# toutane/arcanefem

Measured on AMD Instinct MI355X. Metric: MDoF/s assembly + CG iter/s, Poisson-3D P1 at 1/2/4/8 MI355X, higher is better.
Workload: dtype f64; 1 GPU; C2 Poisson-3D P1; n=215, dof_total=10077696, nnz_rank0=150048286, parallelism=z-slab x1, RCCL halo + all-reduce in CG

## Files before the change

arcanefem_amd/_capi.py:

```python
from __future__ import annotations

import ctypes
import os

_HERE = os.path.dirname(os.path.abspath(__file__))
LIB_PATH = os.environ.get("AFEM_LIB") or os.path.join(_HERE, "libafem.so")

AFEM_OK = 0
AFEM_MEM_HOST = 0
AFEM_MEM_DEVICE = 1
AFEM_RHS_ADD = 0
AFEM_RHS_SET = 1
AFEM_SOLVER_AUTO = 0
AFEM_SOLVER_PCG = 1
AFEM_SOLVER_DIRECT = 2
AFEM_NEUMANN_VALUE = 0
AFEM_NEUMANN_NORMAL = 1
AFEM_NEUMANN_TRACTION = 2
UNIQUE_ID_BYTES = 128
ERRORS = {1: "ArgumentException", 2: "HipError", 3: "NotImplementedException", 4: "StateError",
          5: "NotFound", 6: "CommError", 7: "LimitExceeded"}


class AfemError(RuntimeError):
# ... 25 lines not shown
                ("coords", ctypes.c_void_p), ("rows", ctypes.c_void_p), ("columns", ctypes.c_void_p),
                ("values", ctypes.c_void_p), ("error_flag", ctypes.c_void_p), ("stream", ctypes.c_void_p)]


class FunctorPlan(ctypes.Structure):
    _fields_ = [("n_units", ctypes.c_int64), ("n_stages", ctypes.c_int64), ("n_entries", ctypes.c_int64),
                ("rows_per_layer", ctypes.c_int32), ("width", ctypes.c_int32), ("nbuf", ctypes.c_int32),
                ("wide", ctypes.c_int32), ("block_size", ctypes.c_int32), ("nb_node_per_cell", ctypes.c_int32),
                ("ordered_per_block", ctypes.c_int32), ("lattice", ctypes.c_int32), ("units", ctypes.c_void_p),
                ("stage_ptr", ctypes.c_void_p), ("layer_rows", ctypes.c_void_p), ("entries", ctypes.c_void_p),
                ("entries2", ctypes.c_void_p), ("rows", ctypes.c_void_p), ("values", ctypes.c_void_p),
                ("stream", ctypes.c_void_p), ("patterns", ctypes.c_void_p), ("n_patterns", ctypes.c_int64),
                ("packed", ctypes.c_int32), ("reserved0", ctypes.c_int32)]


class Csr32View(ctypes.Structure):
    _fields_ = [("n_rows", ctypes.c_int64), ("nnz", ctypes.c_int64), ("rows", ctypes.c_void_p),
                ("rows_nb_column", ctypes.c_void_p), ("columns", ctypes.c_void_p), ("values", ctypes.c_void_p),
                ("identity", ctypes.c_int32)]


class BsrStats(ctypes.Structure):
    _fields_ = [("n_incidences", ctypes.c_int64), ("inc_table_entries", ctypes.c_int64),
                ("max_row_len", ctypes.c_int32), ("rows_per_block", ctypes.c_int32), ("max_seg", ctypes.c_int64),
                ("max_slice_nodes", ctypes.c_int32), ("max_slice_width", ctypes.c_int32),
                ("n_slices", ctypes.c_int64), ("brick_order", ctypes.c_int32), ("uniform_slices", ctypes.c_int32),
                ("last_kernel", ctypes.c_int32), ("stencil_slices", ctypes.c_int32),
                ("stencil_sig", ctypes.c_int32), ("shared_strip_slices", ctypes.c_int64),
                ("uniform_instance_slices", ctypes.c_int64), ("general_slices", ctypes.c_int64),
                ("cube_lattice", ctypes.c_int32), ("cube_axes", ctypes.c_int32),
                ("cube_row_stride", ctypes.c_int64), ("cube_units", ctypes.c_int64),
                ("cube_unit_records", ctypes.c_int64), ("cube_unit_table", ctypes.c_void_p),
                ("cube_xcd_cost_spread", ctypes.c_double), ("cube_sched", ctypes.c_int32),
                ("reserved0", ctypes.c_int32)]


class SolverOpts(ctypes.Structure):
    _fields_ = [("method", ctypes.c_int32), ("max_iter", ctypes.c_int32), ("rtol", ctypes.c_double),
                ("atol", ctypes.c_double), ("check_every", ctypes.c_int32), ("fixed_iterations", ctypes.c_int32),
                ("initial_guess", ctypes.c_int32), ("precond_block", ctypes.c_int32), ("multigrid", ctypes.c_int32),
                ("profile_comm", ctypes.c_int32), ("amg", ctypes.c_int32)]


class SolveStats(ctypes.Structure):
    _fields_ = [("iterations", ctypes.c_int32), ("converged", ctypes.c_int32), ("rel_residual", ctypes.c_double),
                ("residual_norm", ctypes.c_double), ("solve_ms", ctypes.c_double), ("spmv_kernel", ctypes.c_int32),
                ("halo_wait_ms", ctypes.c_double), ("allreduce_ms", ctypes.c_double), ("halo_bytes", ctypes.c_int64),
                ("n_halo", ctypes.c_int32), ("n_allreduce", ctypes.c_int32), ("amg_levels", ctypes.c_int32),
                ("amg_coarse_rows", ctypes.c_int64), ("amg_complexity", ctypes.c_double),
                ("amg_setup_ms", ctypes.c_double), ("precond_ms", ctypes.c_double)]


class StepTiming(ctypes.Structure):
    _fields_ = [("assemble_ms", ctypes.c_double), ("rhs_ms", ctypes.c_double), ("bc_ms", ctypes.c_double),
                ("solve_ms", ctypes.c_double), ("precond_ms", ctypes.c_double), ("update_ms", ctypes.c_double),
                ("total_ms", ctypes.c_double), ("iterations", ctypes.c_int32), ("reserved0", ctypes.c_int32),
                ("nnz_blocks", ctypes.c_int64), ("n_incidences", ctypes.c_int64), ("n_nodes", ctypes.c_int64),
                ("n_own_nodes", ctypes.c_int64)]


ALLREDUCE_FN = ctypes.CFUNCTYPE(ctypes.c_int, ctypes.c_void_p, ctypes.POINTER(ctypes.c_double), ctypes.c_int64)
EXCHANGE_FN = ctypes.CFUNCTYPE(ctypes.c_int, ctypes.c_void_p, ctypes.c_int, ctypes.POINTER(ctypes.c_int32),
                               ctypes.POINTER(ctypes.c_double), ctypes.POINTER(ctypes.c_int64),
                               ctypes.POINTER(ctypes.c_double), ctypes.POINTER(ctypes.c_int64))


class HostTransport(ctypes.Structure):
# ... 144 lines not shown
```

arcanefem_amd/csrc/afem_internal.hpp:

```cpp
#pragma once

#include <hip/hip_runtime.h>

#include <cstdint>
#include <map>
#include <memory>
#include <stdexcept>
#include <string>
#include <thread>
#include <utility>
#include <vector>

#include "../../include/arcanefem_amd.h"

namespace afem {

#ifndef AFEM_NT_STORES
#define AFEM_NT_STORES 0
#endif
template <class T>
__device__ __forceinline__ void st_out(T* p, T v)
{
#if AFEM_NT_STORES
  __builtin_nontemporal_store(v, p);
// ... 165 lines not shown
  int64_t n_msl = 0;
  int msl_nodes = 0;
  int ms_nodes = 0, mb_nodes = 0, mb_w = 0;
  int u_nodes = 0, u_w = 0;
  DevBuf<SliceRec> rec_k, rec_ur;
  DevBuf<uint8_t> urslot;
  DevBuf<SliceRec> rec_k0, rec_u1;
  DevBuf<uint8_t> u1slot;
  int64_t n_k0 = 0, n_u1 = 0;
  int64_t n_k = 0, n_ur = 0;
  int sig_k = -1, k_nodes = 0, ur_nodes = 0, ur_w = 0;
  int64_t n_strip_shared = 0;
  bool rec_ok = false;
  DevBuf<int64_t> pos_rb;
  DevBuf<uint32_t> pos_dl;
  DevBuf<unsigned long long> tickets;
  int64_t ticket_gen = 0;
  int64_t n_slices = 0;
  int64_t n_incidences = 0;
  int max_row_len = 0;
  int64_t max_wave_seg = 0;
  DevBuf<int64_t> diag_pos;
  bool canon = false;
  DevBuf<uint8_t> cperm;
  bool cube_ok = false;
  int64_t cube_L[3] = { 0, 0, 0 };
  bool cube_natural = false;
  int nat_axes[3] = { 0, 1, 2 };
  int64_t nat_L[3] = { 0, 0, 0 };
  int64_t cube_row_stride = 0;
  DevBuf<uint32_t> cube_units;
  int64_t cube_units_n = 0, cube_units_real = 0;
  int cube_units_sched = 0;
  double cube_xcd_spread = 0.0;
  int64_t cube_units_key[12] = { 0, 0, 0, 0, 0, 0, 0, 0, 0, 0, 0, 0 };
  DevBuf<int32_t> cube_phys;
  DevBuf<int64_t> cube_rb;
  DevBuf<uint64_t> cube_slot;
  DevBuf<int32_t> cube_lat;
  DevBuf<uint64_t> cube_pinv;
};

struct LinearSystem;

struct FunctorPlan {
  bool valid = false;
  int nb_dof = 0;
  int rl = 64, w = 0, nbuf = 1, wide = 0, lattice = 0;
  int fx = 0, fy = 0, zs = 1;
  int64_t n_units = 0, n_stages = 0, n_entries = 0, n_coalesced = 0;
  DevBuf<afem_functor_unit> units;
  DevBuf<int64_t> stage_ptr;
  DevBuf<int32_t> layer_rows;
  DevBuf<uint32_t> ent, ent2;
  int packed = 0;
  int64_t n_patterns = 0;
  DevBuf<uint32_t> patterns;
};
void functor_plan_build(struct Bsr& b);

struct HandOver {
  bool valid = false, identity = false;
  int64_t n_rows = 0, nnz = 0;
  DevBuf<int32_t> rows, rnc, cols;
  DevBuf<int64_t> src;
  DevBuf<double> vals;
};

// ... 232 lines not shown
```

arcanefem_amd/csrc/capi.cpp:

```cpp
#include <hip/hip_runtime.h>

#include <algorithm>
#include <cstring>
#include <string>
#include <vector>

#include <rocprofiler-sdk-roctx/roctx.h>

#include "afem_internal.hpp"

using namespace afem;

namespace {
thread_local std::string g_last_error;

int fail(int code, const char* msg)
{
  g_last_error = msg ? msg : "unknown error";
  return code;
}
}

#define API_BEGIN try {
#define API_END                                              \
// ... 634 lines not shown
  API_END
}

int afem_bsr_get_stats(afem_bsr* b, afem_bsr_stats* st)
{
  API_BEGIN
  NOT_NULL(b);
  NOT_NULL(st);
  AFEM_REQUIRE(b->has_sparsity, AFEM_ERR_STATE, "no sparsity");
  st->n_incidences = b->s.n_incidences;
  st->inc_table_entries = (int64_t)b->s.inc.n;
  st->max_row_len = b->s.max_row_len;
  st->rows_per_block = afem::assembly_uses_lds(*b) ? 64 : 0;
  st->max_seg = b->s.max_wave_seg;
  st->max_slice_nodes = b->s.max_slice_nodes;
  st->max_slice_width = b->s.max_slice_w;
  st->n_slices = b->s.n_slices;
  st->brick_order = b->s.lattice ? 2 : b->s.brick_order ? 1 : 0;
  st->cube_lattice = b->s.cube_natural ? 2 : (b->s.canon && b->s.cube_ok) ? 3
                     : (b->mesh->st.valid && b->mesh->st.dim == 3 && !b->s.canon) ? 1 : 0;
  st->uniform_slices = (int32_t)b->s.n_uni;
  st->stencil_slices = (int32_t)b->s.n_k;
  st->stencil_sig = b->s.sig_k;
  st->shared_strip_slices = b->s.n_strip_shared;
  st->uniform_instance_slices = b->s.n_ur;
  st->general_slices = b->s.n_ms + b->s.n_mb;
  st->cube_axes = b->s.cube_natural ? b->s.nat_axes[0] + 3 * b->s.nat_axes[1] + 9 * b->s.nat_axes[2] : 0;
  st->cube_row_stride = b->s.cube_row_stride;
  st->cube_units = b->s.cube_units_real;
  st->cube_unit_records = b->s.cube_units_n;
  st->cube_unit_table = b->s.cube_units.p;
  st->cube_xcd_cost_spread = b->s.cube_xcd_spread;
  st->cube_sched = b->s.cube_units_sched;
  st->reserved0 = 0;
  st->last_kernel = b->last_kernel;
  API_END
}

int afem_bsr_get_sizes(afem_bsr* b, int64_t* n_rows, int64_t* nnz)
{
  API_BEGIN
  NOT_NULL(b);
  AFEM_REQUIRE(b->has_sparsity, AFEM_ERR_STATE, "no sparsity");
  if (n_rows) *n_rows = b->s.n_rows * b->nb_dof;
  if (nnz) *nnz = b->s.nnz * b->nb_dof * b->nb_dof;
  API_END
}

int afem_bsr_download(afem_bsr* b, int64_t* rows, int32_t* cols, double* vals)
{
  API_BEGIN
  NOT_NULL(b);
  AFEM_REQUIRE(b->has_sparsity, AFEM_ERR_STATE, "no sparsity");
  Ctx& ctx = *b->mesh->ctx;
  ctx.set_device();
  if (rows) AFEM_HIP(hipMemcpyAsync(rows, b->s.row_ptr.p, b->s.row_ptr.bytes(), hipMemcpyDeviceToHost, ctx.stream));
  if (cols && b->s.nnz)
    AFEM_HIP(hipMemcpyAsync(cols, b->s.cols.p, (size_t)b->s.nnz * sizeof(int32_t), hipMemcpyDeviceToHost, ctx.stream));
  if (vals && b->values.n)
    AFEM_HIP(hipMemcpyAsync(vals, b->values.p, b->values.bytes(), hipMemcpyDeviceToHost, ctx.stream));
  ctx.sync();
  API_END
}

int afem_bsr_export_csr32(afem_bsr* b, int32_t* rows, int32_t* rows_nb_column, int32_t* columns, double* values)
{
  API_BEGIN
// ... 869 lines not shown
```

arcanefem_amd/csrc/cubes.hip:

```cpp
#include "afem_internal.hpp"

#include <algorithm>
#include <cstring>
#include <limits>
#include <vector>

#pragma clang diagnostic ignored "-Wpass-failed"

namespace afem {

namespace {

inline unsigned grid_for(int64_t n, int threads) { return (unsigned)((n + threads - 1) / threads); }

struct P3 {
  double x, y, z;
};
__device__ __forceinline__ P3 psub(P3 a, P3 b) { return P3{ a.x - b.x, a.y - b.y, a.z - b.z }; }
__device__ __forceinline__ P3 pcross(P3 a, P3 b)
{
  return P3{ fma(a.y, b.z, -(a.z * b.y)), fma(a.z, b.x, -(a.x * b.z)), fma(a.x, b.y, -(a.y * b.x)) };
}
__device__ __forceinline__ double pdot(P3 a, P3 b) { return fma(a.z, b.z, fma(a.y, b.y, a.x * b.x)); }
__device__ __forceinline__ double precip(double a)
// ... 99 lines not shown
constexpr int kCol = 9;
constexpr int kAcc = 15;

#ifndef AFEM_CUBES_WAVESYNC
#define AFEM_CUBES_WAVESYNC 1
#endif
__device__ __forceinline__ void wave_lds_order()
{
#if AFEM_CUBES_WAVESYNC
  __builtin_amdgcn_fence(__ATOMIC_ACQ_REL, "wavefront");
  __builtin_amdgcn_wave_barrier();
#else
  __syncthreads();
#endif
}

template <bool NT>
__device__ __forceinline__ void put(double* p, double v)
{
  if constexpr (NT)
    __builtin_nontemporal_store(v, p);
  else
    *p = v;
}

struct CubeCanon {
  const int32_t* phys;
  const int64_t* rb;
  const uint64_t* slot;
  double* stage;
};

constexpr int kCubesBase = 16 | 32 | 64 | 256 | 512 | 1024 | 2048;
constexpr int kCubesV = kCubesBase | 4096;

template <int STRIDE>
constexpr int cube_waves() { return STRIDE == 64 ? 2 : 3; }
template <int STRIDE, bool CARRY, bool XEX, bool YEX, bool CANON, bool HAS_RHS, bool RHS_ADD, int DIAG = kCubesV>
__global__ __launch_bounds__(64) __attribute__((amdgpu_waves_per_eu(cube_waves<STRIDE>(), cube_waves<STRIDE>()))) void k_assemble_cubes(
    CubeGeom g, const int64_t* __restrict__ rows, const double* __restrict__ coords, double* __restrict__ vals,
    double* __restrict__ rhs, CubeCanon cc)
{
  __shared__ __align__(16) double acc[2][kAcc][STRIDE];
  constexpr int NCZ = CARRY ? 1 : 2;
  __shared__ double cz[NCZ][3][kCol * kCol];
  const int lane = threadIdx.x;
  const uint2 rec = g.units[blockIdx.x];
  const int z0 = (int)(rec.y & 0xffffffu), z1 = z0 + (int)(rec.y >> 24);
  if (z0 >= z1) return;
  AFEM_CWT(0, __builtin_amdgcn_s_memrealtime());
  const int cx0 = kRun * (int)(rec.x & 0xffffu), cy0 = kRun * (int)(rec.x >> 16);
  const int zc_first = max(z0 - 1, 0);
  const int zc_last = min(z1 - 1, g.nzc - 1);

  const int ci = lane & 7, cj = lane >> 3;
  const int gx = cx0 - 1 + ci, gy = cy0 - 1 + cj;
  const bool cube_in = gx >= 0 && gy >= 0 && gx + 1 < g.npx && gy + 1 < g.npy;
  auto node_xy = [&](int q, int& nx, int& ny) {
    nx = cx0 - 1 + q % kCol;
    ny = cy0 - 1 + q / kCol;
  };
  double pre[2][3];
  int32_t pid[2] = { 0, 0 };
  auto layer_base = [&](int k) { return (int64_t)__builtin_amdgcn_readfirstlane(local_layer(g, k)) * g.L; };
  int64_t xy_id[2];
#pragma unroll
  for (int h = 0; h < 2; ++h) {
    const int q = min(lane + 64 * h, kCol * kCol - 1);
    int nx, ny;
    node_xy(q, nx, ny);
    nx = min(max(nx, 0), g.npx - 1);
    ny = min(max(ny, 0), g.npy - 1);
    xy_id[h] = nx + (int64_t)g.npx * ny;
  }
  auto clamp_layer = [&](int k) { return is_local(g, k) ? k : g.k0; };
  auto prefetch_ids = [&](int k) {
    if constexpr (CANON) {
      const int32_t* const lp = cc.phys + layer_base(clamp_layer(k));
#pragma unroll
      for (int h = 0; h < 2; ++h) pid[h] = lp[xy_id[h]];
    }
  };
  auto load_layer_to = [&](int k, double (&dst)[2][3]) {
    const double* const lc = CANON ? coords : coords + 3 * layer_base(clamp_layer(k));
#pragma unroll
    for (int h = 0; h < 2; ++h) {
      const int64_t n = CANON ? (int64_t)pid[h] : xy_id[h];
      dst[h][0] = lc[3 * n];
      dst[h][1] = lc[3 * n + 1];
      dst[h][2] = lc[3 * n + 2];
    }
  };
  auto load_layer = [&](int k) { load_layer_to(k, pre); };
  auto store_layer = [&](int buf) {
    buf = NCZ == 1 ? 0 : buf;
#pragma unroll
    for (int h = 0; h < 2; ++h) {
      const int q = min(lane + 64 * h, kCol * kCol - 1);
      cz[buf][0][q] = pre[h][0];
      cz[buf][1][q] = pre[h][1];
      cz[buf][2][q] = pre[h][2];
    }
  };
  constexpr bool DROWS = (DIAG & 256) != 0 && STRIDE == 64;
  constexpr bool SW = DROWS && CARRY && XEX && YEX && (DIAG & 2048) != 0 && (DIAG & 2) == 0;
  auto slot = [&](int b, int r, int o) -> double* {
    return SW ? &acc[b][0][0] + kAcc * r + o : &acc[b][o][r];
  };
  if (!SW || g.acc_init != g.acc_init) {
    const double fill = SW ? g.acc_init : 0.0;
    for (int i = lane; i < 2 * kAcc * STRIDE; i += 64) (&acc[0][0][0])[i] = fill;
  }

  const int rx = lane % kRun, ry = lane / kRun;
  const int nx = cx0 + rx, ny = cy0 + ry;
  const bool full_flush_on = g.full_flush != 0;
  constexpr bool STAGE = CANON && (DIAG & 1024) != 0;
  int64_t pf_rb = 0, pf_re = 0, pf_r = 0;
  uint64_t pf_slot = 0;
  double pf_rhs = 0.0;
  const int64_t row_xy = min(nx, g.npx - 1) + (int64_t)g.npx * min(ny, g.npy - 1);
  auto prefetch_rows = [&](int z) {
    const int zz = (z >= z0 && z < z1) ? z : z0;
    const int64_t lb = layer_base(zz);
    const int64_t li = lb + row_xy;
    if constexpr (STAGE) {
      (void)li;
    }
    else if constexpr (CANON) {
      pf_r = cc.phys[li];
      pf_rb = cc.rb[li];
      pf_slot = cc.slot[li];
    }
    else {
      pf_r = li;
      pf_rb = (rows + lb)[row_xy];
      pf_re = (rows + lb)[row_xy + 1];
      if constexpr (RHS_ADD) pf_rhs = rhs[pf_r];
    }
  };
  const bool xy_full = cx0 >= 1 && cx0 + kRun <= g.npx - 1 && cy0 >= 1 && cy0 + kRun <= g.npy - 1;
  auto full_range = [&](int zlo, int zhi, int& zf0, int& zf1) {
    const bool on = !CANON && xy_full && full_flush_on;
    zf0 = on ? min(max(zlo, g.k0 + 1), zhi) : zhi;
    zf1 = on ? max(min(zhi, g.nzc), zf0) : zhi;
  };
  constexpr bool RS = !CANON && (DIAG & 4096) != 0;
  int64_t rs_rb = 0;
  auto load_run_bases = [&](int z) {
    const int zz = (z >= z0 && z < z1) ? z : z0;
    rs_rb = (rows + layer_base(zz))[row_xy];
  };
  auto flush_full = [&](int z, double* const* sb) {
    const int b = z & 1;
    const int lr = min(lane, STRIDE - 1);
    double v[15];
    double sum = 0.0;
#pragma unroll
    for (int o = 0; o < 15; ++o) {
      v[o] = *slot(b, lr, o);
      if (o != 7) sum += v[o];
    }
    const double meas = v[7];
    v[7] = -sum;
    if constexpr (HAS_RHS) {
      const bool valid = lane < kRows;
      const double rv = RHS_ADD ? pf_rhs + g.f_meas * meas : g.f_meas * meas;
      const int64_t r0 = lane_i64(pf_r, 0);
      const double rv0 = lane_f64(rv, 0);
      put<(DIAG & 128) != 0>(&rhs[valid ? pf_r : r0], valid ? rv : rv0);
    }
    const int64_t rb = pf_rb;
    double* img = &acc[b][0][0];
    if constexpr (SW) {
      img[kAcc * lane + 7] = v[7];
    }
    else {
      wave_lds_order();
#pragma unroll
      for (int o = 0; o < 15; ++o) img[15 * (STRIDE == 64 ? lane : lr) + o] = v[o];
// ... 17 lines not shown
      }
      else if constexpr ((DIAG & 64) != 0) {
        const double a0 = ra[q][0], a1 = ra[q][1];
        typedef double d2u __attribute__((ext_vector_type(2), aligned(8)));
        if constexpr ((DIAG & 32) != 0)
          __builtin_nontemporal_store(d2u{ a0, a1 }, reinterpret_cast<d2u*>(&dst[t2]));
        else
          *reinterpret_cast<d2u*>(&dst[t2]) = d2u{ a0, a1 };
      }
      else if constexpr ((DIAG & 32) != 0) {
        __builtin_nontemporal_store(img[15 * kRun * q + lane], &dst[lane]);
        __builtin_nontemporal_store(img[15 * kRun * q + t1], &dst[t1]);
      }
      else {
        dst[lane] = img[15 * kRun * q + lane];
        dst[t1] = img[15 * kRun * q + t1];
      }
    }
    wave_lds_order();
    if constexpr (SW) {
    }
    else if constexpr ((kAcc * STRIDE) % 2 == 0) {
      double2* const img2 = reinterpret_cast<double2*>(img);
#pragma unroll
      for (int i = 0; i < (kAcc * STRIDE / 2 + 63) / 64; ++i)
        img2[min(64 * i + lane, kAcc * STRIDE / 2 - 1)] = make_double2(0.0, 0.0);
      wave_lds_order();
    }
    else {
#pragma unroll
      for (int i = 0; i < (kAcc * STRIDE + 63) / 64; ++i) img[min(64 * i + lane, kAcc * STRIDE - 1)] = 0.0;
      wave_lds_order();
    }
  };
  auto flush_stage = [&](int z) {
    const int b = z & 1;
    const bool valid = lane < kRows && nx < g.npx && ny < g.npy;
    uint32_t mask = 0;
#pragma unroll
    for (int o = 0; o < 15; ++o) {
      const int xx = nx + kOffX[o], yy = ny + kOffY[o], zz = z + kOffZ[o];
      const uint32_t in = (uint32_t)(xx >= 0) & (uint32_t)(yy >= 0) & (uint32_t)(xx < g.npx) & (uint32_t)(yy < g.npy) &
                          (uint32_t)(zz >= 0) & (uint32_t)(zz <= g.nzc);
      mask |= in << o;
    }
    if (!valid) mask = 0;
    double v[15];
    double sum = 0.0;
    const int lr = min(lane, STRIDE - 1);
#pragma unroll
    for (int o = 0; o < 15; ++o) {
      v[o] = *slot(b, lr, o);
      if (o != 7 && ((mask >> o) & 1u)) sum += v[o];
    }
    const double meas = v[7];
    v[7] = -sum;
    wave_lds_order();
    double* img = &acc[b][0][0];
    if (lane < kRows) {
#pragma unroll
      for (int o = 0; o < 15; ++o) img[16 * lane + o] = (!SW || o == 7 || ((mask >> o) & 1u)) ? v[o] : 0.0;
      img[16 * lane + 15] = meas;
    }
    wave_lds_order();
    typedef double d2u __attribute__((ext_vector_type(2), aligned(16)));
    const int64_t lz = (int64_t)local_layer(g, z) * g.L + cx0;
// ... 221 lines not shown
        atomicAdd(slot_d(bb, bt, c, 7), cm[c - 4]);
      else
        atomicAdd(base_at(inm, bb, bt, c) + STRIDE * 7, kept(c, cm[c - 4]));
    }
  };
  P3 Xc[4];
  auto prime_corners = [&](int zc) {
#pragma unroll
    for (int c = 0; c < 4; ++c) {
      const int q = (ci + cbit(c, 0)) + kCol * (cj + cbit(c, 1));
      const int bz = NCZ == 1 ? 0 : (zc & 1);
      Xc[c] = P3{ cz[bz][0][q], cz[bz][1][q], cz[bz][2][q] };
    }
  };
  auto cubes = [&](int zc) {
    const int bb = zc & 1, bt = (zc + 1) & 1;
    P3 X[8];
#pragma unroll
    for (int c = 0; c < 4; ++c) {
      const int q = (ci + cbit(c, 0)) + kCol * (cj + cbit(c, 1));
      const int zb = NCZ == 1 ? 0 : bb, zt = NCZ == 1 ? 0 : bt;
      X[c] = CARRY ? Xc[c] : P3{ cz[zb][0][q], cz[zb][1][q], cz[zb][2][q] };
      X[c + 4] = P3{ cz[zt][0][q], cz[zt][1][q], cz[zt][2][q] };
      if constexpr (CARRY) Xc[c] = X[c + 4];
    }
    double ev[8][8];
    double mv[8];
#pragma unroll
    for (int a = 0; a < 8; ++a) {
      mv[a] = 0.0;
#pragma unroll
      for (int b = 0; b < 8; ++b) ev[a][b] = 0.0;
    }
#pragma unroll
    for (int t = 0; t < ((DIAG & 4) ? 0 : 6); ++t) {
      const int v1 = tet_v(t, 1), v2 = tet_v(t, 2);
      const P3 e1 = psub(X[v1], X[0]), e2 = psub(X[v2], X[0]), e3 = psub(X[7], X[0]);
      P3 k[4];
      k[1] = pcross(e2, e3);
      k[2] = pcross(e3, e1);
      k[3] = pcross(e1, e2);
      k[0] = P3{ -(k[1].x + k[2].x + k[3].x), -(k[1].y + k[2].y + k[3].y), -(k[1].z + k[2].z + k[3].z) };
      const double meas = cube_in ? fabs(pdot(e1, k[1])) : 0.0;
      const double s = cube_in ? g.s_coef * precip(fmax(meas, 1e-300)) : 0.0;
#pragma unroll
      for (int p = 0; p < 4; ++p) {
        mv[tet_v(t, p)] += meas;
#pragma unroll
        for (int q = p + 1; q < 4; ++q) {
          const int a = tet_v(t, p) < tet_v(t, q) ? tet_v(t, p) : tet_v(t, q);
          const int b = tet_v(t, p) < tet_v(t, q) ? tet_v(t, q) : tet_v(t, p);
          ev[a][b] += s * pdot(k[p], k[q]);
        }
      }
    }
    if constexpr (CARRY) {
      ev[0][1] += ce[0];
      ev[0][2] += ce[1];
      ev[0][3] += ce[2];
      ev[1][3] += ce[3];
      ev[2][3] += ce[4];
#pragma unroll
      for (int c = 0; c < 4; ++c) mv[c] += cm[c];
      ce[0] = ev[4][5];
      ce[1] = ev[4][6];
      ce[2] = ev[4][7];
      ce[3] = ev[5][7];
      ce[4] = ev[6][7];
#pragma unroll
      for (int c = 0; c < 4; ++c) cm[c] = mv[c + 4];
    }
    if constexpr (YEX) {
      ev[2][3] += __shfl_down(ev[0][1], 8);
      ev[2][6] += __shfl_down(ev[0][4], 8);
      ev[2][7] += __shfl_down(ev[0][5], 8);
      ev[3][7] += __shfl_down(ev[1][5], 8);
      mv[2] += __shfl_down(mv[0], 8);
// ... 96 lines not shown
    next_layer(zc + 2);
    wave_lds_order();
    cubes(zc);
    wave_lds_order();
    if constexpr (DROWS && !SW) {
      double2* const b2 = reinterpret_cast<double2*>(&acc[zc & 1][0][0]);
#pragma unroll
      for (int i = 0; i < (kAcc * STRIDE / 2 + 63) / 64; ++i)
        b2[min(64 * i + lane, kAcc * STRIDE / 2 - 1)] = make_double2(0.0, 0.0);
      wave_lds_order();
    }
    store_layer(zc & 1);
    settle_ids();
    ++zc;
  }
  auto layer_step = [&](int zc, auto&& fl) {
    prefetch_rows(zc);
    if constexpr ((DIAG & 16) != 0) next_layer(zc + 2);
    wave_lds_order();
    cubes(zc);
    if constexpr ((DIAG & 16) == 0) next_layer(zc + 2);
    wave_lds_order();
    fl(zc);
    store_layer(zc & 1);
  };
#pragma nounroll
  for (int ph = 0; ph < 2; ++ph) {
    const int zend = ph == 0 ? zf0 : zc_last + 1;
#pragma nounroll
    for (; zc < zend; ++zc) layer_step(zc, flush);
    if constexpr (!CANON) {
      if (ph == 0) {
        if constexpr (RS) {
          if (g.row_stride != 0) {
#pragma nounroll
            for (; zc < zf1; ++zc) {
              pf_r = layer_base(zc) + row_xy;
              if constexpr (RHS_ADD) pf_rhs = rhs[pf_r];
              if constexpr ((DIAG & 16) != 0) next_layer(zc + 2);
              wave_lds_order();
              cubes(zc);
              if constexpr ((DIAG & 16) == 0) next_layer(zc + 2);
              wave_lds_order();
              if constexpr (!(DIAG & 8)) flush_full(zc, run_base);
              store_layer(zc & 1);
#pragma unroll
              for (int q = 0; q < kRun; ++q) run_base[q] += g.row_stride;
            }
          }
        }
#pragma nounroll
        for (; zc < zf1; ++zc)
          layer_step(zc, [&](int z) {
            if constexpr (!(DIAG & 8)) flush_full(z, nullptr);
          });
      }
    }
  }
  if (zc_last + 1 >= z0 && zc_last + 1 < z1) {
    prefetch_rows(zc_last + 1);
    if constexpr (CARRY) {
      add_top(zc_last);
      wave_lds_order();
    }
    flush(zc_last + 1);
  }
  AFEM_CWT(1, __builtin_amdgcn_s_memrealtime());
}

__global__ void k_cube_stage_maps(int64_t n, int npx, int npy, int nzc, const int32_t* __restrict__ phys,
                                  const uint64_t* __restrict__ slot, int32_t* __restrict__ lat,
                                  uint64_t* __restrict__ pinv)
{
  const int64_t i = (int64_t)blockIdx.x * blockDim.x + threadIdx.x;
  if (i >= n) return;
  const int64_t L = (int64_t)npx * npy;
  const int z = (int)(i / L);
  const int64_t rem = i - (int64_t)z * L;
  const int y = (int)(rem / npx), x = (int)(rem - (int64_t)y * npx);
  uint32_t mask = 0;
  for (int o = 0; o < 15; ++o) {
    const int xx = x + kOffX[o], yy = y + kOffY[o], zz = z + kOffZ[o];
    if (xx >= 0 && yy >= 0 && xx < npx && yy < npy && zz >= 0 && zz <= nzc) mask |= 1u << o;
  }
  const uint64_t sl = slot[i];
  uint64_t w = 0;
  for (int o = 0; o < 15; ++o)
    if ((mask >> o) & 1u) {
      const int t = __popc(mask & ((1u << o) - 1u));
      const int pos = (int)((sl >> (4 * t)) & 15u);
      w |= (uint64_t)o << (4 * pos);
    }
// ... 88 lines not shown
  const bool natural = S.cube_natural;
  canon = !natural && S.canon && S.cube_ok;
  if (!canon && !natural && (!st.valid || st.dim != 3 || S.canon || st.lx > 0 || st.ly > 0 || st.n < 1)) return false;
  if (canon || natural) {
    const int64_t* Lc = natural ? S.nat_L : S.cube_L;
    g.npx = (int)Lc[0];
    g.npy = (int)Lc[1];
    g.nzc = (int)Lc[2] - 1;
    g.k0 = 0;
    g.k1 = (int)Lc[2];
    g.ghost_lo = g.ghost_hi = -1;
    g.L = Lc[0] * Lc[1];
  }
  else {
    g.npx = g.npy = st.n + 1;
    g.nzc = st.nz;
    g.k0 = st.k0;
    g.k1 = st.k1;
    g.ghost_lo = st.ghost_lo;
    g.ghost_hi = st.ghost_hi;
    g.L = st.L;
    if (g.L != (int64_t)g.npx * g.npy) return false;
  }
  g.n_own_layers = g.k1 - g.k0;
  if (g.n_own_layers <= 0 || g.nzc < 1 || g.npx < 2 || g.npy < 2) return false;
  g.tx = (g.npx + kRun - 1) / kRun;
  g.ty = (g.npy + kRun - 1) / kRun;
  return true;
}

constexpr double kCostStart = 0.62;
constexpr double kCostBelow = 0.81;
constexpr double kCostFull = 1.0;
constexpr double kCostGeneral = 1.67;
constexpr double kCostTop = 0.90;
constexpr int kXcds = 8;

struct CubeUnitWork {
  int below, full, general, top;
};
CubeUnitWork cube_unit_work(const CubeGeom& g, bool canon, const CubeUnit& u)
{
  const int cx0 = kRun * u.cx, cy0 = kRun * u.cy;
  const int zc_first = std::max(u.z0 - 1, 0), zc_last = std::min(u.z1 - 1, g.nzc - 1);
  const bool xy_full = cx0 >= 1 && cx0 + kRun <= g.npx - 1 && cy0 >= 1 && cy0 + kRun <= g.npy - 1;
  const int zhi = zc_last + 1;
  int zf0 = zhi, zf1 = zhi;
  if (!canon && xy_full && g.full_flush) {
    zf0 = std::min(std::max(u.z0, g.k0 + 1), zhi);
    zf1 = std::max(std::min(zhi, g.nzc), zf0);
  }
  CubeUnitWork w;
  w.below = zc_first < u.z0 ? 1 : 0;
  w.full = zf1 - zf0;
  w.general = std::max(zhi - u.z0, 0) - w.full;
  w.top = (zhi >= u.z0 && zhi < u.z1) ? 1 : 0;
  return w;
}
double cube_unit_cost(const CubeGeom& g, bool canon, const CubeUnit& u)
{
  const CubeUnitWork w = cube_unit_work(g, canon, u);
  return kCostStart + kCostBelow * w.below + kCostFull * w.full + kCostGeneral * w.general + kCostTop * w.top;
}

void build_cube_units(const Mesh& m, Structure& S, const CubeGeom& g, bool canon, int sched, int band_rows,
                      const std::vector<int>& pat)
{
  int64_t pat_key = 0;
  for (int p : pat) pat_key = pat_key * 256 + p;
  const int64_t key[12] = { g.npx, g.npy, g.nzc, g.k0, g.k1, pat_key, (int64_t)pat.size(),
                            band_rows, g.n_own_layers, canon ? 1 : 0, g.full_flush, sched };
  if (S.cube_units.p && std::equal(key, key + 12, S.cube_units_key)) return;
  std::vector<int> cuts{ g.k0 };
  for (size_t i = 0; cuts.back() < g.k1; ++i) cuts.push_back(std::min(cuts.back() + pat[i % pat.size()], g.k1));
  const int64_t n_col = (int64_t)g.tx * g.ty, n_units = n_col * (int64_t)(cuts.size() - 1);
  AFEM_REQUIRE(n_units < (int64_t(1) << 31), AFEM_ERR_LIMIT, "cube kernel: too many units");
  std::vector<CubeUnit> units((size_t)n_units);
  std::vector<double> cost((size_t)n_units);
  double total = 0.0;
  for (int64_t u = 0; u < n_units; ++u) {
    const int seg = (int)(u / n_col);
    units[u] = CubeUnit{ (int32_t)(u % g.tx), (int32_t)((u / g.tx) % g.ty), cuts[seg], cuts[seg + 1] };
    cost[u] = cube_unit_cost(g, canon, units[u]);
    total += cost[u];
  }
  std::vector<int64_t> list[kXcds];
  if (sched) {
    double cum = 0.0;
    for (int64_t u = 0; u < n_units; ++u) {
      const int x = std::min(kXcds - 1, (int)(kXcds * (cum + 0.5 * cost[u]) / total));
      list[x].push_back(u);
      cum += cost[u];
    }
    const int64_t band = band_rows > 0 ? (int64_t)band_rows * g.tx : n_units;
    for (auto& l : list)
      std::stable_sort(l.begin(), l.end(), [&](int64_t a, int64_t b) {
        return a / band != b / band ? a / band < b / band : cost[a] > cost[b];
      });
  }
  else {
    const int64_t qq = n_units / kXcds, rem = n_units % kXcds;
    for (int x = 0; x < kXcds; ++x) {
      const int64_t first = x * qq + std::min<int64_t>(x, rem), count = qq + (x < rem ? 1 : 0);
      for (int64_t j = 0; j < count; ++j) list[x].push_back(first + j);
    }
  }
  size_t longest = 0;
  double cmax = 0.0, cmin = std::numeric_limits<double>::max();
  for (const auto& l : list) {
    longest = std::max(longest, l.size());
    if (l.empty()) continue;
    double c = 0.0;
    for (int64_t u : l) c += cost[u];
    cmax = std::max(cmax, c);
    cmin = std::min(cmin, c);
  }
  const int64_t n_rec = sched ? (int64_t)kXcds * (int64_t)longest : n_units;
  AFEM_REQUIRE(n_rec < (int64_t(1) << 31), AFEM_ERR_LIMIT, "cube kernel: too many units");
  AFEM_REQUIRE(g.tx <= kUnitMaxColumns && g.ty <= kUnitMaxColumns && g.k1 < kUnitMaxLayer,
               AFEM_ERR_LIMIT, "cube kernel: a unit does not fit its record");
  auto packed = [](const CubeUnit& u) {
    return uint2{ (uint32_t)u.cx | (uint32_t)u.cy << 16, (uint32_t)u.z0 | (uint32_t)(u.z1 - u.z0) << 24 };
  };
  std::vector<uint2> table((size_t)n_rec, packed(CubeUnit{ 0, 0, g.k0, g.k0 }));
  for (int x = 0; x < kXcds; ++x)
    for (size_t j = 0; j < list[x].size(); ++j) table[kXcds * j + x] = packed(units[list[x][j]]);
  Ctx& ctx = *m.ctx;
  S.cube_units.alloc(2 * (size_t)n_rec);
  AFEM_HIP(hipMemcpyAsync(S.cube_units.p, table.data(), sizeof(uint2) * (size_t)n_rec, hipMemcpyHostToDevice,
                          ctx.stream));
  ctx.sync();
  S.cube_units_n = n_rec;
  S.cube_units_real = n_units;
  S.cube_units_sched = sched;
  S.cube_xcd_spread = cmax / cmin;
  std::copy(key, key + 12, S.cube_units_key);
}

}

void cube_row_stride(const Mesh& m, Structure& S, int nb_dof)
{
  S.cube_row_stride = 0;
  CubeGeom g{};
  bool canon = false;
  if (!cube_lattice_geom(m, S, nb_dof, g, canon) || canon) return;
  const int64_t lmax = std::min(g.k1, g.nzc) - g.k0;
  if (lmax < 2 || lmax * g.L > S.n_rows) return;
  Ctx& ctx = *m.ctx;
  int64_t h[2] = { 0, 0 };
  AFEM_HIP(hipMemcpyAsync(&h[0], S.row_ptr.p + g.L, sizeof(int64_t), hipMemcpyDeviceToHost, ctx.stream));
  AFEM_HIP(hipMemcpyAsync(&h[1], S.row_ptr.p + 2 * g.L, sizeof(int64_t), hipMemcpyDeviceToHost, ctx.stream));
  ctx.sync();
  const int64_t C = h[1] - h[0];
  if (C <= 0) return;
  int32_t bad = 0;
  const int64_t n_pairs = (lmax - 2) * g.L;
  if (n_pairs > 0) {
    DevBuf<int32_t> flag;
    flag.alloc(1);
    AFEM_HIP(hipMemsetAsync(flag.p, 0, flag.bytes(), ctx.stream));
    hipLaunchKernelGGL(k_row_stride_check, dim3(grid_for(n_pairs, 256)), dim3(256), 0, ctx.stream, S.row_ptr.p, g.L,
                       (int64_t)1, lmax - 1, C, flag.p);
    AFEM_LAUNCHED();
    AFEM_HIP(hipMemcpyAsync(&bad, flag.p, sizeof(bad), hipMemcpyDeviceToHost, ctx.stream));
    ctx.sync();
  }
  S.cube_row_stride = bad ? 0 : C;
}

bool assemble_cubes(Bsr& b, double coef, double f, double* rhs, int rhs_add)
{
  const Mesh& m = *b.mesh;
  Structure& S = b.s;
  const char* ce = variant("AFEM_ASSEMBLY_CUBES");
  if (ce && atoi(ce) == 0) return false;
  CubeGeom g{};
  bool canon = false;
  if (!cube_lattice_geom(m, S, b.nb_dof, g, canon)) return false;
  Ctx& ctx = *m.ctx;
  g.row_stride = S.cube_row_stride;
  const char* ze = variant("AFEM_CUBES_ZS");
  std::vector<int> pat;
  for (const char* p = ze; p && *p && pat.size() < 7; p = strchr(p, '/') ? strchr(p, '/') + 1 : "")
    pat.push_back(std::min(kUnitMaxLayers, std::max(1, atoi(p))));
  if (pat.empty()) pat.push_back(std::min(48, std::max(8, std::max(g.npx, g.npy) / 16)));
  g.zs = *std::max_element(pat.begin(), pat.end());
  g.ns = 0;
  g.s_coef = coef / 6.0;
  g.f_meas = f / 24.0;
  const char* fe = variant("AFEM_CUBES_FULL");
  g.full_flush = (fe && atoi(fe) == 0) ? 0 : 1;
  const char* ie = variant("AFEM_CUBES_ACC_INIT");
  g.acc_init = (ie && (ie[0] == 'n' || ie[0] == 'N')) ? std::numeric_limits<double>::quiet_NaN() : 0.0;
  const char* sce = variant("AFEM_CUBES_SCHED");
  const char* be = variant("AFEM_CUBES_BAND");
  build_cube_units(m, S, g, canon, (sce && atoi(sce) == 0) ? 0 : 1, be ? std::max(0, atoi(be)) : 0, pat);
  g.units = reinterpret_cast<const uint2*>(S.cube_units.p);
  const char* se = variant("AFEM_CUBES_STRIDE");
  const bool s49 = se && atoi(se) == 49;
  const char* ke = variant("AFEM_CUBES_CARRY");
  const bool carry = canon || !(ke && atoi(ke) == 0);
  const char* xe = variant("AFEM_CUBES_XEX");
  const bool xex = canon || (carry && !(xe && atoi(xe) == 0));
  const char* ye = variant("AFEM_CUBES_YEX");
  const bool yex = canon || (xex && !(ye && atoi(ye) == 0));
#define AFEM_CUBES_K(S, C, X, Y, N, D)                                                                               \
  (rhs ? (rhs_add ? &k_assemble_cubes<S, C, X, Y, N, true, true, D> : &k_assemble_cubes<S, C, X, Y, N, true, false, D>) \
       : &k_assemble_cubes<S, C, X, Y, N, false, false, D>)
  const char* de = variant("AFEM_CUBES_V");
  const int diag = de ? atoi(de) : kCubesV;
  constexpr int kB = kCubesBase;
  auto* kern = canon ? AFEM_CUBES_K(64, true, true, true, true, kB & ~1024)
               : carry ? (xex ? (yex ? (s49 ? AFEM_CUBES_K(49, true, true, true, false, kB)
                                            : ((diag & 4096) ? AFEM_CUBES_K(64, true, true, true, false, kB | 4096)
                                                             : AFEM_CUBES_K(64, true, true, true, false, kB)))
                                     : AFEM_CUBES_K(64, true, true, false, false, kB))
                              : AFEM_CUBES_K(64, true, false, false, false, kB))
                       : (s49 ? AFEM_CUBES_K(49, false, false, false, false, kB)
                              : AFEM_CUBES_K(64, false, false, false, false, kB));
#undef AFEM_CUBES_K
  if (diag != (kB | 4096) && diag != kB && carry && xex && yex && rhs && !rhs_add) {
    switch (diag) {
#define AFEM_CUBES_D(D)                                                                                              \
  case D:                                                                                                            \
    kern = canon ? &k_assemble_cubes<64, true, true, true, true, true, false, (D) & ~(1024 | 4096)>                 \
                 : &k_assemble_cubes<64, true, true, true, false, true, false, D>;                                  \
    break;
      AFEM_CUBES_D(0) AFEM_CUBES_D(112) AFEM_CUBES_D(kB | 1) AFEM_CUBES_D(kB | 4)
      AFEM_CUBES_D(kB | 8) AFEM_CUBES_D(kB | 2) AFEM_CUBES_D(kB & ~512) AFEM_CUBES_D(kB & ~1024)
      AFEM_CUBES_D(kB & ~32) AFEM_CUBES_D(kB & ~2048) AFEM_CUBES_D(kB & ~(1024 | 2048))
      AFEM_CUBES_D(kB | 4096 | 1) AFEM_CUBES_D(kB | 4096 | 4) AFEM_CUBES_D(kB | 4096 | 8)
#undef AFEM_CUBES_D
      default: break;
    }
  }
  CubeCanon cc{ canon ? S.cube_phys.p : nullptr, canon ? S.cube_rb.p : nullptr, canon ? S.cube_slot.p : nullptr,
                nullptr };
  const int64_t n_lat = g.L * (int64_t)(g.nzc + 1);
  const bool staged = canon && (diag & 1024) != 0 && n_lat == S.n_rows;
  if (staged) {
    if (S.cube_lat.n != (size_t)n_lat) {
      S.cube_lat.alloc(n_lat);
      S.cube_pinv.alloc(n_lat);
      hipLaunchKernelGGL(k_cube_stage_maps, dim3(grid_for(n_lat, 256)), dim3(256), 0, ctx.stream, n_lat, g.npx, g.npy,
                         g.nzc, S.cube_phys.p, S.cube_slot.p, S.cube_lat.p, S.cube_pinv.p);
      AFEM_LAUNCHED();
    }
    if (b.cube_stage.n != (size_t)(16 * n_lat)) b.cube_stage.alloc(16 * n_lat);
    cc.stage = b.cube_stage.p;
    kern = &k_assemble_cubes<64, true, true, true, true, false, false, kCubesBase | 1024>;
    if (diag != (kCubesBase | 4096) && diag != kCubesBase) {
      switch (diag) {
#define AFEM_CUBES_S(D)                                                                                              \
  case D:                                                                                                            \
    kern = &k_assemble_cubes<64, true, true, true, true, false, false, D>;                                          \
    break;
        AFEM_CUBES_S(kCubesBase | 1024 | 1) AFEM_CUBES_S(kCubesBase | 1024 | 4) AFEM_CUBES_S(kCubesBase & ~2048)
#undef AFEM_CUBES_S
        default: break;
      }
    }
  }
  hipLaunchKernelGGL(kern, dim3((unsigned)S.cube_units_n), dim3(64), 0, ctx.stream, g, S.row_ptr.p, m.coords.p,
                     b.values.p, rhs, cc);
  AFEM_LAUNCHED();
  if (staged) {
    const int64_t n = S.n_rows;
    auto* un = rhs ? (rhs_add ? &k_cube_unstage<true, true> : &k_cube_unstage<true, false>)
                   : &k_cube_unstage<false, false>;
    const char* uve = variant("AFEM_UNSTAGE_V");
    const int uv = uve ? atoi(uve) : 3;
    if (rhs && !rhs_add && uv == 0) un = &k_cube_unstage<true, false, 0>;
    if (rhs && !rhs_add && uv == 1) un = &k_cube_unstage<true, false, 1>;
    if (rhs && !rhs_add && uv == 2) un = &k_cube_unstage<true, false, 2>;
    hipLaunchKernelGGL(un, dim3((unsigned)grid_for(n, 64)), dim3(64), 0, ctx.stream, n, S.row_ptr.p, S.cube_lat.p,
                       S.cube_pinv.p, b.cube_stage.p, g.f_meas, b.values.p, rhs);
    AFEM_LAUNCHED();
  }
  b.last_kernel = AFEM_KERNEL_CUBES;
  return true;
}

}
```

include/arcanefem_amd.h:

```cpp
#ifndef ARCANEFEM_AMD_H
#define ARCANEFEM_AMD_H

#include <stddef.h>
#include <stdint.h>

#ifdef __cplusplus
extern "C" {
#endif

#define AFEM_OK 0
#define AFEM_ERR_ARG 1
#define AFEM_ERR_HIP 2
#define AFEM_ERR_NOT_IMPL 3
#define AFEM_ERR_STATE 4
#define AFEM_ERR_NOT_FOUND 5
#define AFEM_ERR_COMM 6
#define AFEM_ERR_LIMIT 7

#define AFEM_MEM_HOST 0
#define AFEM_MEM_DEVICE 1

typedef struct afem_ctx afem_ctx;
typedef struct afem_mesh afem_mesh;
typedef struct afem_bsr afem_bsr;
// ... 67 lines not shown
int afem_bsr_assemble_poisson_p1_ex(afem_bsr* bsr, double coef, double f, double* rhs, int rhs_mode);
int afem_bsr_assemble_elasticity_p1(afem_bsr* bsr, double lambda, double mu2);
int afem_bsr_assemble_elasticity_p1_ex(afem_bsr* bsr, double lambda, double mu2, double mass_coef,
                                       const double* body_force, double* rhs, int rhs_mode);
int afem_bsr_reset_values(afem_bsr* bsr);
int afem_bsr_set_value(afem_bsr* bsr, int32_t row, int32_t col, double v);
int afem_bsr_get_value(afem_bsr* bsr, int32_t row, int32_t col, double* v);
int afem_bsr_view(afem_bsr* bsr, afem_csr_view* view);
typedef struct afem_bsr_stats {
  int64_t n_incidences;
  int64_t inc_table_entries;
  int32_t max_row_len;
  int32_t rows_per_block;
  int64_t max_seg;
  int32_t max_slice_nodes;
  int32_t max_slice_width;
  int64_t n_slices;
  int32_t brick_order;
  int32_t uniform_slices;
  int32_t last_kernel;
  int32_t stencil_slices;
  int32_t stencil_sig;
  int64_t shared_strip_slices;
  int64_t uniform_instance_slices;
  int64_t general_slices;
  int32_t cube_lattice;
  int32_t cube_axes;
  int64_t cube_row_stride;
  int64_t cube_units;
  int64_t cube_unit_records;
  const uint32_t* cube_unit_table;
  double cube_xcd_cost_spread;
  int32_t cube_sched;
  int32_t reserved0;
} afem_bsr_stats;
#define AFEM_KERNEL_NONE 0
#define AFEM_KERNEL_STRIP 1
#define AFEM_KERNEL_SLICE_TILE 2
#define AFEM_KERNEL_GLOBAL 3
#define AFEM_KERNEL_ELAST3_STRIP 4
#define AFEM_KERNEL_ELAST3_ITEM 5
#define AFEM_KERNEL_ELAST3_GLOBAL 6
#define AFEM_KERNEL_ELAST2 7
#define AFEM_KERNEL_ELAST3_WG 8
#define AFEM_KERNEL_ELAST3_BIG 9
#define AFEM_KERNEL_CUBES 10
int afem_bsr_get_stats(afem_bsr* bsr, afem_bsr_stats* stats);
int afem_bsr_get_sizes(afem_bsr* bsr, int64_t* n_scalar_rows, int64_t* nnz_scalar);
int afem_bsr_export_csr32(afem_bsr* bsr, int32_t* rows, int32_t* rows_nb_column, int32_t* columns, double* values);
typedef struct afem_assembly_view {
  int64_t n_rows;
  int64_t n_nodes;
  int64_t n_cells;
  int32_t nb_node_per_cell;
  int32_t block_size;
  int32_t ordered_per_block;
  int32_t dim;
  const int32_t* cell_node;
  const double* coords;
  const int64_t* rows;
  const int32_t* columns;
  double* values;
  int32_t* error_flag;
  void* stream;
} afem_assembly_view;
int afem_bsr_assembly_view(afem_bsr* bsr, afem_assembly_view* view);
typedef struct afem_functor_unit {
// ... 194 lines not shown
```

Measured before the change: 26470 MDoF/s.

## Add face-unit flush path for boundary cube columns in assembly kernel

Adds a specialized flush path for cube units on the xy domain boundary, which previously fell back to the slower general per-layer path. It builds an LDS permutation table once per unit that maps accumulator entries to compacted CSR row positions, then streams each z-layer with paired nontemporal stores. The boundary-cell mask is also made branchless by multiplying with a 0/1 double. The unit cost model gains a face category so the XCD scheduler rebalances work. This adds LDS use, register pressure and a new kernel variant, which becomes the default.

```diff
diff --git a/arcanefem_amd/_capi.py b/arcanefem_amd/_capi.py
--- a/arcanefem_amd/_capi.py
+++ b/arcanefem_amd/_capi.py
@@ -81,7 +81,7 @@
                 ("cube_row_stride", ctypes.c_int64), ("cube_units", ctypes.c_int64),
                 ("cube_unit_records", ctypes.c_int64), ("cube_unit_table", ctypes.c_void_p),
                 ("cube_xcd_cost_spread", ctypes.c_double), ("cube_sched", ctypes.c_int32),
-                ("reserved0", ctypes.c_int32)]
+                ("cube_face_plan", ctypes.c_int32)]
 
 
 class SolverOpts(ctypes.Structure):
diff --git a/arcanefem_amd/csrc/afem_internal.hpp b/arcanefem_amd/csrc/afem_internal.hpp
--- a/arcanefem_amd/csrc/afem_internal.hpp
+++ b/arcanefem_amd/csrc/afem_internal.hpp
@@ -221,8 +221,9 @@
   DevBuf<uint32_t> cube_units;
   int64_t cube_units_n = 0, cube_units_real = 0;
   int cube_units_sched = 0;
+  int cube_units_face = 0;
   double cube_xcd_spread = 0.0;
-  int64_t cube_units_key[12] = { 0, 0, 0, 0, 0, 0, 0, 0, 0, 0, 0, 0 };
+  int64_t cube_units_key[13] = { 0, 0, 0, 0, 0, 0, 0, 0, 0, 0, 0, 0, 0 };
   DevBuf<int32_t> cube_phys;
   DevBuf<int64_t> cube_rb;
   DevBuf<uint64_t> cube_slot;
diff --git a/arcanefem_amd/csrc/capi.cpp b/arcanefem_amd/csrc/capi.cpp
--- a/arcanefem_amd/csrc/capi.cpp
+++ b/arcanefem_amd/csrc/capi.cpp
@@ -690,7 +690,7 @@
   st->cube_unit_table = b->s.cube_units.p;
   st->cube_xcd_cost_spread = b->s.cube_xcd_spread;
   st->cube_sched = b->s.cube_units_sched;
-  st->reserved0 = 0;
+  st->cube_face_plan = b->s.cube_units_face;
   st->last_kernel = b->last_kernel;
   API_END
 }
diff --git a/arcanefem_amd/csrc/cubes.hip b/arcanefem_amd/csrc/cubes.hip
--- a/arcanefem_amd/csrc/cubes.hip
+++ b/arcanefem_amd/csrc/cubes.hip
@@ -155,7 +155,8 @@
 };
 
 constexpr int kCubesBase = 16 | 32 | 64 | 256 | 512 | 1024 | 2048;
-constexpr int kCubesV = kCubesBase | 4096;
+constexpr int kCubesFace = 16384;
+constexpr int kCubesV = kCubesBase | 4096 | kCubesFace;
 
 template <int STRIDE>
 constexpr int cube_waves() { return STRIDE == 64 ? 2 : 3; }
@@ -179,6 +180,7 @@
   const int ci = lane & 7, cj = lane >> 3;
   const int gx = cx0 - 1 + ci, gy = cy0 - 1 + cj;
   const bool cube_in = gx >= 0 && gy >= 0 && gx + 1 < g.npx && gy + 1 < g.npy;
+  uint32_t in_hi = cube_in ? 0x3ff00000u : 0u;
   auto node_xy = [&](int q, int& nx, int& ny) {
     nx = cx0 - 1 + q % kCol;
     ny = cy0 - 1 + q / kCol;
@@ -242,7 +244,7 @@
   int64_t pf_rb = 0, pf_re = 0, pf_r = 0;
   uint64_t pf_slot = 0;
   double pf_rhs = 0.0;
-  const int64_t row_xy = min(nx, g.npx - 1) + (int64_t)g.npx * min(ny, g.npy - 1);
+  int64_t row_xy = min(nx, g.npx - 1) + (int64_t)g.npx * min(ny, g.npy - 1);
   auto prefetch_rows = [&](int z) {
     const int zz = (z >= z0 && z < z1) ? z : z0;
     const int64_t lb = layer_base(zz);
@@ -263,12 +265,16 @@
     }
   };
   const bool xy_full = cx0 >= 1 && cx0 + kRun <= g.npx - 1 && cy0 >= 1 && cy0 + kRun <= g.npy - 1;
+  constexpr bool RS = !CANON && (DIAG & 4096) != 0;
+  constexpr bool FP = RS && SW && (DIAG & kCubesFace) != 0;
+  const bool face_unit = FP && !xy_full && g.row_stride != 0;
+  constexpr int kPlanRow = 15 * kRun + 1;
+  __shared__ unsigned short ptab[FP ? kRun * kPlanRow : 2];
   auto full_range = [&](int zlo, int zhi, int& zf0, int& zf1) {
-    const bool on = !CANON && xy_full && full_flush_on;
+    const bool on = !CANON && (xy_full || face_unit) && full_flush_on;
     zf0 = on ? min(max(zlo, g.k0 + 1), zhi) : zhi;
     zf1 = on ? max(min(zhi, g.nzc), zf0) : zhi;
   };
-  constexpr bool RS = !CANON && (DIAG & 4096) != 0;
   int64_t rs_rb = 0;
   auto load_run_bases = [&](int z) {
     const int zz = (z >= z0 && z < z1) ? z : z0;
@@ -352,6 +358,42 @@
       for (int i = 0; i < (kAcc * STRIDE + 63) / 64; ++i) img[min(64 * i + lane, kAcc * STRIDE - 1)] = 0.0;
       wave_lds_order();
     }
+  };
+  auto flush_face = [&](int z, double* const* sb, const uint32_t (&ps)[kRun], bool valid) {
+    const int b = z & 1;
+    double* img = &acc[b][0][0];
+    double v[15];
+    double sum = 0.0;
+#pragma unroll
+    for (int o = 0; o < 15; ++o) {
+      v[o] = img[kAcc * lane + o];
+      if (o != 7) sum += v[o];
+    }
+    const double meas = v[7];
+    if constexpr (HAS_RHS) {
+      const double rv = RHS_ADD ? pf_rhs + g.f_meas * meas : g.f_meas * meas;
+      const int64_t r0 = lane_i64(pf_r, 0);
+      const double rv0 = lane_f64(rv, 0);
+      put<(DIAG & 128) != 0>(&rhs[valid ? pf_r : r0], valid ? rv : rv0);
+    }
+    img[kAcc * lane + 7] = -sum;
+    wave_lds_order();
+    typedef double d2u __attribute__((ext_vector_type(2), aligned(8)));
+    const char* const ib = reinterpret_cast<const char*>(img);
+    d2u w[kRun];
+    uint32_t to[kRun];
+#pragma unroll
+    for (int q = 0; q < kRun; ++q) {
+      uint32_t pq = ps[q];
+      asm volatile("" : "+v"(pq));
+      w[q] = d2u{ *reinterpret_cast<const double*>(ib + (pq & 0x1ff8u)),
+                  *reinterpret_cast<const double*>(ib + ((pq >> 10) & 0x1ff8u)) };
+      to[q] = (pq >> 20) & 0x3f8u;
+    }
+#pragma unroll
+    for (int q = 0; q < kRun; ++q)
+      __builtin_nontemporal_store(w[q], reinterpret_cast<d2u*>(reinterpret_cast<char*>(sb[q]) + to[q]));
+    wave_lds_order();
   };
   auto flush_stage = [&](int z) {
     const int b = z & 1;
@@ -639,6 +681,9 @@
 #pragma unroll
       for (int b = 0; b < 8; ++b) ev[a][b] = 0.0;
     }
+    asm volatile("" : "+v"(in_hi));
+    const double in01 = __hiloint2double((int)in_hi, 0);
+    const double s_in = g.s_coef * in01;
 #pragma unroll
     for (int t = 0; t < ((DIAG & 4) ? 0 : 6); ++t) {
       const int v1 = tet_v(t, 1), v2 = tet_v(t, 2);
@@ -648,8 +693,8 @@
       k[2] = pcross(e3, e1);
       k[3] = pcross(e1, e2);
       k[0] = P3{ -(k[1].x + k[2].x + k[3].x), -(k[1].y + k[2].y + k[3].y), -(k[1].z + k[2].z + k[3].z) };
-      const double meas = cube_in ? fabs(pdot(e1, k[1])) : 0.0;
-      const double s = cube_in ? g.s_coef * precip(fmax(meas, 1e-300)) : 0.0;
+      const double meas = fabs(pdot(e1, k[1])) * in01;
+      const double s = s_in * precip(fmax(meas, 1e-300));
 #pragma unroll
       for (int p = 0; p < 4; ++p) {
         mv[tet_v(t, p)] += meas;
@@ -812,7 +857,7 @@
     if constexpr (!CANON) {
       if (ph == 0) {
         if constexpr (RS) {
-          if (g.row_stride != 0) {
+          if (g.row_stride != 0 && !face_unit) {
 #pragma nounroll
             for (; zc < zf1; ++zc) {
               pf_r = layer_base(zc) + row_xy;
@@ -829,6 +874,58 @@
             }
           }
         }
+        if constexpr (FP) {
+          if (face_unit && zc < zf1) {
+            const bool fvalid = lane < kRows && nx < g.npx && ny < g.npy;
+            uint32_t fmask = 0;
+#pragma unroll
+            for (int o = 0; o < 15; ++o) {
+              const int xx = nx + kOffX[o], yy = ny + kOffY[o];
+              const uint32_t in = (uint32_t)(xx >= 0) & (uint32_t)(yy >= 0) & (uint32_t)(xx < g.npx) & (uint32_t)(yy < g.npy);
+              fmask |= in << o;
+            }
+            if (!fvalid) fmask = 0;
+            const int flen = __popc(fmask);
+            int fp = 0;
+#pragma unroll
+            for (int d = 1; d < kRun; ++d) {
+              const int t = __shfl(flen, lane - d);
+              if (rx - d >= 0) fp += t;
+            }
+            if (fvalid) {
+#pragma unroll
+              for (int o = 0; o < 15; ++o)
+                if ((fmask >> o) & 1u)
+                  ptab[kPlanRow * ry + fp + __popc(fmask & ((1u << o) - 1u))] = (unsigned short)(8 * (kAcc * lane + o));
+            }
+            wave_lds_order();
+            uint32_t psrc[kRun];
+            double* face_base[kRun];
+#pragma unroll
+            for (int q = 0; q < kRun; ++q) {
+              const int qs = cy0 + q < g.npy ? q : 0;
+              const int rl = lane_i32(fp + flen, kRun * qs + kRun - 1);
+              const int t2 = max(min(2 * lane, rl - 2), 0);
+              psrc[q] = (uint32_t)ptab[kPlanRow * qs + t2] | (uint32_t)ptab[kPlanRow * qs + t2 + 1] << 10 |
+                        (uint32_t)t2 << 23;
+              face_base[q] = qs == q ? run_base[q] : run_base[0];
+            }
+#pragma nounroll
+            for (; zc < zf1; ++zc) {
+              pf_r = layer_base(zc) + row_xy;
+              if constexpr (RHS_ADD) pf_rhs = rhs[pf_r];
+              if constexpr ((DIAG & 16) != 0) next_layer(zc + 2);
+              wave_lds_order();
+              cubes(zc);
+              if constexpr ((DIAG & 16) == 0) next_layer(zc + 2);
+              wave_lds_order();
+              flush_face(zc, face_base, psrc, fvalid);
+              store_layer(zc & 1);
+#pragma unroll
+              for (int q = 0; q < kRun; ++q) face_base[q] += g.row_stride;
+            }
+          }
+        }
 #pragma nounroll
         for (; zc < zf1; ++zc)
           layer_step(zc, [&](int z) {
@@ -838,6 +935,11 @@
     }
   }
   if (zc_last + 1 >= z0 && zc_last + 1 < z1) {
+    if constexpr (FP) {
+      int l2 = lane;
+      asm volatile("" : "+v"(l2));
+      row_xy = min(cx0 + l2 % kRun, g.npx - 1) + (int64_t)g.npx * min(cy0 + l2 / kRun, g.npy - 1);
+    }
     prefetch_rows(zc_last + 1);
     if constexpr (CARRY) {
       add_top(zc_last);
@@ -992,45 +1094,48 @@
 constexpr double kCostStart = 0.62;
 constexpr double kCostBelow = 0.81;
 constexpr double kCostFull = 1.0;
+constexpr double kCostFace = 1.06;
 constexpr double kCostGeneral = 1.67;
 constexpr double kCostTop = 0.90;
 constexpr int kXcds = 8;
 
 struct CubeUnitWork {
-  int below, full, general, top;
+  int below, full, face, general, top;
 };
-CubeUnitWork cube_unit_work(const CubeGeom& g, bool canon, const CubeUnit& u)
+CubeUnitWork cube_unit_work(const CubeGeom& g, bool canon, bool face, const CubeUnit& u)
 {
   const int cx0 = kRun * u.cx, cy0 = kRun * u.cy;
   const int zc_first = std::max(u.z0 - 1, 0), zc_last = std::min(u.z1 - 1, g.nzc - 1);
   const bool xy_full = cx0 >= 1 && cx0 + kRun <= g.npx - 1 && cy0 >= 1 && cy0 + kRun <= g.npy - 1;
   const int zhi = zc_last + 1;
   int zf0 = zhi, zf1 = zhi;
-  if (!canon && xy_full && g.full_flush) {
+  if (!canon && (xy_full || face) && g.full_flush) {
     zf0 = std::min(std::max(u.z0, g.k0 + 1), zhi);
     zf1 = std::max(std::min(zhi, g.nzc), zf0);
   }
   CubeUnitWork w;
   w.below = zc_first < u.z0 ? 1 : 0;
-  w.full = zf1 - zf0;
-  w.general = std::max(zhi - u.z0, 0) - w.full;
+  w.full = xy_full ? zf1 - zf0 : 0;
+  w.face = xy_full ? 0 : zf1 - zf0;
+  w.general = std::max(zhi - u.z0, 0) - w.full - w.face;
   w.top = (zhi >= u.z0 && zhi < u.z1) ? 1 : 0;
   return w;
 }
-double cube_unit_cost(const CubeGeom& g, bool canon, const CubeUnit& u)
-{
-  const CubeUnitWork w = cube_unit_work(g, canon, u);
-  return kCostStart + kCostBelow * w.below + kCostFull * w.full + kCostGeneral * w.general + kCostTop * w.top;
-}
-
-void build_cube_units(const Mesh& m, Structure& S, const CubeGeom& g, bool canon, int sched, int band_rows,
+double cube_unit_cost(const CubeGeom& g, bool canon, bool face, const CubeUnit& u)
+{
+  const CubeUnitWork w = cube_unit_work(g, canon, face, u);
+  return kCostStart + kCostBelow * w.below + kCostFull * w.full + kCostFace * w.face + kCostGeneral * w.general +
+         kCostTop * w.top;
+}
+
+void build_cube_units(const Mesh& m, Structure& S, const CubeGeom& g, bool canon, bool face, int sched, int band_rows,
                       const std::vector<int>& pat)
 {
   int64_t pat_key = 0;
   for (int p : pat) pat_key = pat_key * 256 + p;
-  const int64_t key[12] = { g.npx, g.npy, g.nzc, g.k0, g.k1, pat_key, (int64_t)pat.size(),
-                            band_rows, g.n_own_layers, canon ? 1 : 0, g.full_flush, sched };
-  if (S.cube_units.p && std::equal(key, key + 12, S.cube_units_key)) return;
+  const int64_t key[13] = { g.npx, g.npy, g.nzc, g.k0, g.k1, pat_key, (int64_t)pat.size(),
+                            band_rows, g.n_own_layers, canon ? 1 : 0, g.full_flush, sched, face ? 1 : 0 };
+  if (S.cube_units.p && std::equal(key, key + 13, S.cube_units_key)) return;
   std::vector<int> cuts{ g.k0 };
   for (size_t i = 0; cuts.back() < g.k1; ++i) cuts.push_back(std::min(cuts.back() + pat[i % pat.size()], g.k1));
   const int64_t n_col = (int64_t)g.tx * g.ty, n_units = n_col * (int64_t)(cuts.size() - 1);
@@ -1041,7 +1146,7 @@
   for (int64_t u = 0; u < n_units; ++u) {
     const int seg = (int)(u / n_col);
     units[u] = CubeUnit{ (int32_t)(u % g.tx), (int32_t)((u / g.tx) % g.ty), cuts[seg], cuts[seg + 1] };
-    cost[u] = cube_unit_cost(g, canon, units[u]);
+    cost[u] = cube_unit_cost(g, canon, face, units[u]);
     total += cost[u];
   }
   std::vector<int64_t> list[kXcds];
@@ -1093,8 +1198,9 @@
   S.cube_units_n = n_rec;
   S.cube_units_real = n_units;
   S.cube_units_sched = sched;
+  S.cube_units_face = face ? 1 : 0;
   S.cube_xcd_spread = cmax / cmin;
-  std::copy(key, key + 12, S.cube_units_key);
+  std::copy(key, key + 13, S.cube_units_key);
 }
 
 }
@@ -1155,8 +1261,6 @@
   g.acc_init = (ie && (ie[0] == 'n' || ie[0] == 'N')) ? std::numeric_limits<double>::quiet_NaN() : 0.0;
   const char* sce = variant("AFEM_CUBES_SCHED");
   const char* be = variant("AFEM_CUBES_BAND");
-  build_cube_units(m, S, g, canon, (sce && atoi(sce) == 0) ? 0 : 1, be ? std::max(0, atoi(be)) : 0, pat);
-  g.units = reinterpret_cast<const uint2*>(S.cube_units.p);
   const char* se = variant("AFEM_CUBES_STRIDE");
   const bool s49 = se && atoi(se) == 49;
   const char* ke = variant("AFEM_CUBES_CARRY");
@@ -1170,9 +1274,15 @@
        : &k_assemble_cubes<S, C, X, Y, N, false, false, D>)
   const char* de = variant("AFEM_CUBES_V");
   const int diag = de ? atoi(de) : kCubesV;
-  constexpr int kB = kCubesBase;
+  constexpr int kB = kCubesBase, kF = kCubesBase | 4096 | kCubesFace;
+  const bool headline = !canon && carry && xex && yex && !s49;
+  const bool face_v = headline && (diag & (4096 | kCubesFace)) == (4096 | kCubesFace);
+  const bool face = face_v && g.row_stride != 0 && g.full_flush;
+  build_cube_units(m, S, g, canon, face, (sce && atoi(sce) == 0) ? 0 : 1, be ? std::max(0, atoi(be)) : 0, pat);
+  g.units = reinterpret_cast<const uint2*>(S.cube_units.p);
   auto* kern = canon ? AFEM_CUBES_K(64, true, true, true, true, kB & ~1024)
                : carry ? (xex ? (yex ? (s49 ? AFEM_CUBES_K(49, true, true, true, false, kB)
+                                            : face_v ? AFEM_CUBES_K(64, true, true, true, false, kF)
                                             : ((diag & 4096) ? AFEM_CUBES_K(64, true, true, true, false, kB | 4096)
                                                              : AFEM_CUBES_K(64, true, true, true, false, kB)))
                                      : AFEM_CUBES_K(64, true, true, false, false, kB))
@@ -1180,7 +1290,7 @@
                        : (s49 ? AFEM_CUBES_K(49, false, false, false, false, kB)
                               : AFEM_CUBES_K(64, false, false, false, false, kB));
 #undef AFEM_CUBES_K
-  if (diag != (kB | 4096) && diag != kB && carry && xex && yex && rhs && !rhs_add) {
+  if (diag != kF && diag != (kB | 4096) && diag != kB && carry && xex && yex && rhs && !rhs_add) {
     switch (diag) {
 #define AFEM_CUBES_D(D)                                                                                              \
   case D:                                                                                                            \
@@ -1210,7 +1320,7 @@
     if (b.cube_stage.n != (size_t)(16 * n_lat)) b.cube_stage.alloc(16 * n_lat);
     cc.stage = b.cube_stage.p;
     kern = &k_assemble_cubes<64, true, true, true, true, false, false, kCubesBase | 1024>;
-    if (diag != (kCubesBase | 4096) && diag != kCubesBase) {
+    if (diag != kF && diag != (kCubesBase | 4096) && diag != kCubesBase) {
       switch (diag) {
 #define AFEM_CUBES_S(D)                                                                                              \
   case D:                                                                                                            \
diff --git a/include/arcanefem_amd.h b/include/arcanefem_amd.h
--- a/include/arcanefem_amd.h
+++ b/include/arcanefem_amd.h
@@ -123,7 +123,7 @@
   const uint32_t* cube_unit_table;
   double cube_xcd_cost_spread;
   int32_t cube_sched;
-  int32_t reserved0;
+  int32_t cube_face_plan;
 } afem_bsr_stats;
 #define AFEM_KERNEL_NONE 0
 #define AFEM_KERNEL_STRIP 1
```

Result: slower. 25150 MDoF/s (-5.0%).
